# openclimatefix/graph_weather

Measured on AMD Instinct MI355X. Metric: forward forecasts/sec (1° grid, 102→78 feat), higher is better.
Workload: dtype f32; 1 GPU; c2: GraphWeatherForecaster 1deg grid (64800 nodes), 102->78 feat, batch=2 on rank 0, fp32, mesh res 2 (5882 nodes), random-init weights; global_batch=2, parallelism=batch-sharded x1, no collective in forward

## Files before the change

### graph_weather_amd/_lib.py

```python
from __future__ import annotations

import ctypes
import os
import subprocess
from ctypes import POINTER, Structure, c_char_p, c_float, c_int, c_int32, c_int64, c_size_t, c_void_p

_HERE = os.path.dirname(os.path.abspath(__file__))
CSRC = os.path.join(_HERE, "csrc")
LIB_PATH = os.path.join(CSRC, "libgw_amd.so")
HIPCC_FLAGS = ["--offload-arch=gfx950", "-O3", "-std=c++17", "-munsafe-fp-atomics", "-shared", "-fPIC"]

ABI_VERSION = 19
DTYPE_F32, DTYPE_BF16, DTYPE_BF16X3 = 0, 1, 2
LAYOUT_ROWS_F32, LAYOUT_EDGE_TILES_BF16, LAYOUT_ROWS_F16, LAYOUT_ROWS_BF16K = 0, 1, 2, 3
EDGE_DETERMINISTIC, EDGE_SEGMENT_TILES, EDGE_AGG_BF16K, EDGE_SEGMENT_SPLIT = 1, 2, 4, 8

EXPORTS = [
    "gw_version", "gw_last_error", "gw_debug_timestamps", "gw_packed_floats", "gw_pack_linear", "gw_packed_bytes_bf16",
    "gw_pack_linear_bf16", "gw_packed_bytes_bf16x3", "gw_pack_linear_bf16x3", "gw_padded_n", "gw_pad_vector", "gw_pack_many", "gw_mlp_chain_backward", "gw_mlp_chain_backward_bf16x3", "gw_mlp_ln_chain_backward",
    "gw_mlp_forward", "gw_mlp_post_forward", "gw_project_forward", "gw_edge_update_forward", "gw_edge_update_workspace_bytes", "gw_edge_tiles_bytes",
    "gw_edge_rows_to_tiles", "gw_node_update_forward", "gw_node_update_row_split_groups", "gw_node_update_head_forward",
    "gw_normalized_mse_forward", "gw_gemm_f32", "gw_relu_backward", "gw_layernorm_backward", "gw_gather_rows",
    "gw_segment_sum_rows", "gw_normalized_mse_backward", "gw_adamw_step", "gw_nudging_forward", "gw_nudging_backward",
    "gw_linear_forward", "gw_linear_gather_forward", "gw_layernorm_forward", "gw_add_rows", "gw_gather_rows_wide", "gw_segment_sum_rows_wide",
# ... 4 lines not shown
    "gw_thermal_rows",
    "gw_amse_mmax", "gw_amse_dft_rows", "gw_amse_legendre_floats", "gw_amse_coeff_floats", "gw_amse_workspace_bytes",
    "gw_amse_forward", "gw_amse_backward",
    "gw_modulate_workspace_bytes", "gw_sdl_forward", "gw_sdl_backward", "gw_film_forward", "gw_film_backward",
    "gw_attention_forward", "gw_attention_backward", "gw_knn_interpolate_forward", "gw_knn_interpolate_backward",
    "gw_gelu_forward", "gw_gelu_backward",
    "gw_attention_axial_forward", "gw_attention_axial_backward",
    "gw_patch_workspace_bytes", "gw_patch_embed_forward", "gw_patch_embed_backward", "gw_patch_expand_forward",
    "gw_patch_expand_backward",
    "gw_attention_masked_forward", "gw_attention_masked_backward",
    "gw_earth_loss_workspace_bytes", "gw_earth_loss_forward", "gw_earth_loss_backward",
    "gw_token_mean_forward", "gw_token_mean_backward", "gw_relu_forward", "gw_row_scale",
    "gw_conv3d_workspace_bytes", "gw_conv3d_forward", "gw_conv3d_backward",
    "gw_gemm_tn_ordered_workspace_bytes", "gw_gemm_tn_ordered", "gw_layernorm_backward_ordered_workspace_bytes",
    "gw_layernorm_backward_ordered",
    "gw_encoder_fused_forward",
    "gw_graph_attention_forward", "gw_graph_attention_backward", "gw_cond_layernorm_forward", "gw_cond_layernorm_backward",
    "gw_beta_gate_forward", "gw_beta_gate_workspace_bytes", "gw_beta_gate_backward", "gw_silu_forward", "gw_silu_backward",
    "gw_fourier_forward", "gw_fourier_backward",
    "gw_graph_attention_batched_forward", "gw_graph_attention_batched_backward", "gw_cond_layernorm_grouped_forward",
    "gw_cond_layernorm_grouped_workspace_bytes", "gw_cond_layernorm_grouped_backward", "gw_gencast_precond_input_forward",
    "gw_gencast_precond_input_backward", "gw_gencast_precond_output_forward", "gw_gencast_precond_output_backward",
    "gw_isht_lmax", "gw_isht_legendre_floats", "gw_isht_workspace_bytes", "gw_isht_forward",
    "gw_gencast_sampler_combine", "gw_gencast_weighted_mse_workspace_bytes", "gw_gencast_weighted_mse_forward",
    "gw_gencast_weighted_mse_backward",
    "gw_cond_layernorm_fanout_forward", "gw_cond_layernorm_fanout_workspace_bytes", "gw_cond_layernorm_fanout_backward",
    "gw_linear_gather_grouped_forward", "gw_segment_sum_rows_grouped",
]

GEMM_NN, GEMM_TN, GEMM_TN_BF16X3 = 0, 1, 2

# ... 145 lines not shown
    L.gw_edge_tiles_bytes.argtypes = [c_int32, c_int32]
    L.gw_edge_rows_to_tiles.restype = c_int
    L.gw_edge_rows_to_tiles.argtypes = [c_int32, c_int32, c_void_p, c_int32, c_int32, c_void_p, c_void_p]
    L.gw_edge_update_workspace_bytes.restype = c_size_t
    L.gw_edge_update_workspace_bytes.argtypes = [c_int32, c_int32, POINTER(GwOperand), POINTER(GwOperand), POINTER(GwOperand),
                                                 POINTER(GwMlpWeights), c_int32]
    L.gw_node_update_forward.restype = c_int
    L.gw_node_update_forward.argtypes = [c_int64, c_int32, POINTER(GwOperand), POINTER(GwOperand), POINTER(GwOperand),
                                         POINTER(GwMlpWeights), c_void_p, c_int32, POINTER(GwActivationSave), c_int32,
                                         POINTER(c_void_p), POINTER(c_void_p), c_int32, c_void_p, c_void_p]
    L.gw_node_update_row_split_groups.restype = c_int
    L.gw_node_update_row_split_groups.argtypes = [c_int64]
    L.gw_node_update_head_forward.restype = c_int
    L.gw_node_update_head_forward.argtypes = [c_int64, c_int32, POINTER(GwOperand), POINTER(GwOperand), POINTER(GwMlpWeights),
                                              POINTER(GwMlpWeights), POINTER(GwOperand), c_void_p, c_int32, c_void_p]
    L.gw_project_forward.restype = c_int
    L.gw_project_forward.argtypes = [c_int64, c_int32, POINTER(GwOperand), c_int32, POINTER(c_void_p), POINTER(c_void_p),
                                     c_int32, c_int32, c_int32, c_void_p, c_void_p, c_void_p]
    L.gw_normalized_mse_forward.restype = c_int
    L.gw_normalized_mse_forward.argtypes = [c_void_p, c_void_p, c_void_p, c_int32, c_void_p, c_int32, c_int32, c_int32, c_int32,
                                            c_void_p, c_void_p]
    L.gw_gemm_f32.restype = c_int
    L.gw_gemm_f32.argtypes = [c_int32, c_int64, c_int32, c_int64, c_void_p, c_int32, c_void_p, c_int32, c_void_p, c_int32, c_void_p,
                              c_void_p]
    L.gw_relu_backward.restype = c_int
    L.gw_relu_backward.argtypes = [c_int64, c_int32, c_void_p, c_int32, c_void_p, c_int32, c_void_p, c_int32, c_void_p, c_void_p]
    L.gw_layernorm_backward.restype = c_int
    L.gw_layernorm_backward.argtypes = [c_int64, c_int32, c_void_p, c_int32, c_void_p, c_int32, c_void_p, c_void_p, c_int32, c_void_p,
                                        c_void_p, c_void_p]
    L.gw_gather_rows.restype = c_int
# ... 264 lines not shown
```

### graph_weather_amd/layers.py

```python
from __future__ import annotations

from typing import List, Optional, Tuple

import torch
from torch import nn

from . import autograd as ag
from . import ops
from . import routes
from . import wide
from .autograd import OperandSpec
from .graphs import ForecastGraphs, GraphPlan, build_forecast_graphs
from .ops import BF16X3, Operand, PackedMLP
from .thermalizer import ThermalizerLayer

_NORMS = ["LayerNorm", "GraphNorm", "InstanceNorm", "BatchNorm", "MessageNorm"]


def _ver(t: torch.Tensor) -> int:
    return -1 if t.is_inference() else t._version


def _version_key(params) -> tuple:
    return tuple((p.data_ptr(), _ver(p), p.device) for p in params)
# ... 19 lines not shown
        hit = self._entries.get(name)
        if hit is None or hit[0] != key or hit[2] is not hold:
            hit = (key, make(), hold)
            self._entries[name] = hit
        return hit[1]

    def fresh(self, name: str, key, hold=None) -> bool:
        hit = self._entries.get(name)
        return hit is not None and hit[0] == key and hit[2] is hold

    def clear(self) -> None:
        self._entries.clear()

    def __contains__(self, name: str) -> bool:
        return name in self._entries


def _autograd_on(module: nn.Module, *inputs: Optional[torch.Tensor]) -> bool:
    on = torch.is_grad_enabled() and (any(p.requires_grad for p in module.parameters())
                                      or any(t is not None and t.requires_grad for t in inputs))
    if on:
        for m in module.modules():
            if isinstance(m, MLP) and m.compute_dtype == torch.bfloat16:
                raise NotImplementedError("graph_weather_amd: the backward pass is implemented for float32 and bf16x3 matrix "
                                          "products; call the bfloat16 mode under torch.no_grad() (inference)")
    return on


def _form(mlp: "MLP") -> routes.MlpForm:
    if mlp.compute_dtype == torch.bfloat16:
# ... 208 lines not shown
        self.node_mlp = MLP(in_dim_node + in_dim_edge, in_dim_node, hidden_dim, hidden_layers, norm_type).as_table()
        self.node_mlp.set_input_splits(((0, in_dim_node), (in_dim_node, in_dim_node + in_dim_edge)))


class GraphNetBlock(nn.Module):

    def __init__(self, edge_model: EdgeProcessor, node_model: NodeProcessor):
        super().__init__()
        self.edge_model = edge_model
        self.node_model = node_model
        self.deterministic = False

    def run(self, batch: int, plan: GraphPlan, x_src: Feed, x_dst: Feed, e_in: Feed, e_res: torch.Tensor, e_res_rows_pb: int,
            x_node: Feed, x_res: Optional[torch.Tensor], x_res_rows_pb: int, want_edges: bool, device,
            tag: Optional[str] = None, agg_zeroed: Optional[torch.Tensor] = None, post_w=None, post_zero: bool = False,
            post_half: bool = False, head=None, seg=None, agg_acc: Optional[torch.Tensor] = None):
        n_dst, n_edges = plan.n_dst, plan.num_edges
        if _autograd_on(self, x_src.tensor, x_dst.tensor, e_in.tensor, e_res, x_node.tensor, x_res):
            agg, e_out = ag.edge_update(self.edge_model.edge_mlp, plan, batch, (x_src.spec(), x_dst.spec(), e_in.spec()),
                                        want_edges, x_src.tensor, x_dst.tensor, e_in.tensor, e_res, e_res_rows_pb)
            x_new = ag.node_update(self.node_model.node_mlp, batch * n_dst, n_dst, x_node.spec(), x_node.tensor, x_res,
                                   x_res_rows_pb, agg)
            return x_new, e_out
        if seg is not None and agg_acc is not None:
            if want_edges not in (False, "tiles"):
                raise RuntimeError("graph_weather_amd: a processor block on segment-aligned tiles hands e' over as edge tiles")
            agg = agg_acc
            n_edges = seg.n_pad
        elif seg is not None:
            if want_edges or e_res is not None:
                raise RuntimeError("graph_weather_amd: segment-aligned tiles come without residual and without e'")
            if seg.split:
                agg = agg_zeroed if agg_zeroed is not None else torch.zeros((batch * n_dst, 256), dtype=torch.float32, device=device)
            else:
                agg = (torch.empty if seg.complete else torch.zeros)((batch * n_dst, 256), dtype=torch.bfloat16, device=device)
        else:
            agg = agg_zeroed if agg_zeroed is not None else torch.zeros((batch * n_dst, 256), dtype=torch.float32, device=device)
        if want_edges == "tiles":
            e_out = torch.empty(ops.edge_tiles_bytes(batch, n_edges), dtype=torch.uint8, device=device)
        else:
            e_out = torch.empty((batch * n_edges, 256), dtype=torch.float32, device=device) if want_edges else None
        res_op = ops.ZERO if e_res is None else Operand(e_res, e_res_rows_pb, 256, tiles=(e_res.dtype == torch.uint8))
        ops.edge_update_forward(self.edge_model.edge_mlp.packed(), batch, plan.src if seg is None else seg.src,
                                plan.dst if seg is None else seg.dst, x_src.operand(), x_dst.operand(),
                                e_in.operand(), res_op, n_dst, agg, e_out, tag=tag, deterministic=self.deterministic,
                                segment_tiles=seg is not None, segment_split=seg is not None and seg.split and agg_acc is None)
        res_x = ops.ZERO if x_res is None else Operand(x_res, x_res_rows_pb, 256)
        if head is not None:
            if x_res is not None:
                raise RuntimeError("graph_weather_amd: the fused node update + head has no node residual (decoder rows are zeros)")
            y = ops.node_update_head_forward(self.node_model.node_mlp.packed(), head[0], batch * n_dst, n_dst, x_node.operand(),
                                             Operand(agg, n_dst, 256), head[1])
            return y, e_out
        if post_w is not None:
            next_agg = torch.empty((batch * n_dst, 256), dtype=torch.float32, device=device) if post_zero else None
            if seg is not None and agg_acc is not None and not post_zero:
                next_agg = None
            x_new, posts = ops.node_update_forward(self.node_model.node_mlp.packed(), batch * n_dst, n_dst, x_node.operand(), res_x,
                                                   Operand(agg, n_dst, 256), post_w=post_w, zero_rows=next_agg, post_half=post_half)
            return x_new, e_out, posts, next_agg
        x_new = ops.node_update_forward(self.node_model.node_mlp.packed(), batch * n_dst, n_dst, x_node.operand(), res_x,
                                        Operand(agg, n_dst, 256))
        return x_new, e_out

    def params_key(self) -> tuple:
# ... 503 lines not shown
        self.efficient_batching = efficient_batching
        self.num_latlons = len(lat_lons)
        self.graphs = _graphs if _graphs is not None else build_forecast_graphs(lat_lons, resolution)
        self.num_h3 = self.graphs.num_mesh
        self.output_dim = output_dim
        self.edge_encoder = MLP(2, output_edge_dim, hidden_dim_processor_edge, 2, mlp_norm_type, use_checkpointing).as_table()
        self.graph_processor = GraphProcessor(mp_iterations=1, in_dim_node=input_dim, in_dim_edge=output_edge_dim,
                                              hidden_dim_node=hidden_dim_processor_node,
                                              hidden_dim_edge=hidden_dim_processor_edge,
                                              hidden_layers_node=hidden_layers_processor_node,
                                              hidden_layers_edge=hidden_layers_processor_edge, norm_type=mlp_norm_type,
                                              use_checkpointing=use_checkpointing)
        self.node_decoder = MLP(input_dim, output_dim, hidden_dim_decoder, hidden_layers_decoder, None, use_checkpointing)
        self._dev_plans = {}
        self._cache = KeyedCache()

    def _plan(self, device) -> GraphPlan:
        key = str(device)
        if key not in self._dev_plans:
            self._dev_plans[key] = self.graphs.dec_plan.to(device)
        return self._dev_plans[key]

    def edge_embedding(self, plan: GraphPlan) -> torch.Tensor:
        if _autograd_on(self):
            return self.edge_encoder.table(plan.edge_attr)
        return self._cache.get("dec_e", _version_key(list(self.edge_encoder.parameters())), lambda: self.edge_encoder.table(plan.edge_attr))

    def prefetch_tables(self, dev) -> Optional["torch.cuda.Stream"]:
        if wide.decoder_is_wide(self) or _autograd_on(self) or len(self.graph_processor.blocks) == 0:
            return None
# ... 44 lines not shown
            return False
        native = not mlp_e._layout()[4] and mlp_e._norm() is not None and len(mlp_e._linears()) == 3
        form = routes.MlpForm(torch.float32, 1 if native else -1, 0 if native else -1, native)
        return routes.decoder_stream(form, mlp_n.compute_dtype, self.graphs.dec_plan.num_edges, False, _autograd_on(self),
                                     bool(blk.deterministic), bool(ops.EDGE_STREAM))

    def _e_sum_product(self, plan: GraphPlan, e_rows: torch.Tensor, key, half: bool) -> torch.Tensor:
        pm_n = self.graph_processor.blocks[0].node_model.node_mlp.packed()
        n_e = plan.num_edges

        def make_e_sum():
            e_sum = ag.segment_sum_rows(e_rows, n_e, 1, 1, plan.n_dst, plan.dst_ptr(), None)
            return ops.project_forward([pm_n.w1[1]], Operand(e_sum, plan.n_dst, 256), plan.n_dst, plan.n_dst, out_half=half)[0]

        return self._cache.get("dec_e_sum", key, make_e_sum)

    def split_path(self) -> bool:
        return self._block_route() == routes.BLOCK_SPLIT

    def decode(self, processor_features: torch.Tensor, batch_size: int,
               residual: Optional[torch.Tensor] = None, ps: Optional[torch.Tensor] = None) -> torch.Tensor:
        B, G, M = batch_size, self.num_latlons, self.num_h3
        if processor_features.shape[0] != B * M:
            raise RuntimeError("processor_features must have batch*num_h3 rows")
        dev = processor_features.device
        if wide.decoder_is_wide(self):
            return wide.decode(self, processor_features, B, residual=residual)
        processor_features = _pad256(processor_features)
        plan = self._plan(dev)
        e = self.edge_embedding(plan)
# ... 31 lines not shown
        res = None
        if residual is not None:
            if residual.dim() != 2 or residual.shape[0] != B * G or residual.shape[1] < self.output_dim:
                raise RuntimeError("graph_weather_amd: the residual (start features) must have batch*num_latlons rows of at least "
                                   "output_dim = %d features, got %s" % (self.output_dim, tuple(residual.shape)))
            res = Operand(residual, G, self.output_dim)
        head = None
        if not train:
            nd = self.node_decoder
            if nd.compute_dtype == blk.node_model.node_mlp.compute_dtype and not wide.is_wide(nd) and not nd._layout()[4]:
                pm_h = nd.packed()
                pm_nn = blk.node_model.node_mlp.packed()
                if (pm_h.hidden == 128 and pm_h.n_mid == 1 and pm_h.n_out <= 80 and pm_h.gamma is None and pm_nn.n_mid == 1
                        and pm_nn.gamma is not None and pm_nn.ln_width == 0):
                    head = (pm_h, res)
        if not train and x_node is not FEED_ZERO:
            out, _ = blk.run(B, plan, Feed(ps, M, "proj"), FEED_ZERO, Feed(pe, 0, "proj"), None, 0, x_node, None, 0, False, dev,
                             tag="decoder_edge", head=head, seg=seg)
            if head is not None:
                return out.reshape(B, G, self.output_dim)
            xg = out
        elif head is not None and mlp_e.compute_dtype == torch.float32:
            out, _ = blk.run(B, plan, Feed(ps, M, "proj"), FEED_ZERO, Feed(pe, 0, "proj"), e, 0, FEED_ZERO, None, 0, False, dev,
                             tag="decoder_edge", head=head)
            return out.reshape(B, G, self.output_dim)
        else:
            xg, _ = blk.run(B, plan, Feed(ps, M, "proj"), FEED_ZERO, Feed(pe, 0, "proj"), e, 0, FEED_ZERO, None, 0, False, dev,
                            tag="decoder_edge")
        y = self.node_decoder.run(xg, B * G, G, residual=res)
        if y.shape[1] != self.output_dim:
            y = y[:, :self.output_dim]
        return y.reshape(B, G, self.output_dim)

    def forward(self, processor_features: torch.Tensor, batch_size: int) -> torch.Tensor:
        return self.decode(processor_features, batch_size)


def fused_forward(encoder: "Encoder", processor: "Processor", decoder: "AssimilatorDecoder", features: torch.Tensor,
                  residual: torch.Tensor, t=0) -> torch.Tensor:
# ... 77 lines not shown
```

### graph_weather_amd/ops.py

```python
from __future__ import annotations

from dataclasses import dataclass
from typing import List, Optional, Sequence, Tuple

import torch

from . import _lib
from ._lib import GwActivationSave, GwMlpWeights, GwOperand


class KernelTimer:

    def __init__(self, tags):
        self.tags = set(tags)
        self.events = {t: [] for t in self.tags}
        self.units = {t: [] for t in self.tags}

    def start(self, tag):
        if tag not in self.tags:
            return None
        ev = (torch.cuda.Event(enable_timing=True), torch.cuda.Event(enable_timing=True))
        ev[0].record()
        return ev

# ... 11 lines not shown
        evs = self.events[tag]
        return sum(a.elapsed_time(b) for a, b in evs) / max(1, len(evs))


TIMER: Optional[KernelTimer] = None

EDGE_STREAM = True
"""float32 inference: the decoder's edge update runs without the per-edge residual on the decoder-form kernel of
csrc/gw_edge_stream.hip (the segment sums of the batch-shared edge embedding enter the node update as a cached product).
``False`` forces the per-edge residual route on ``edge_kernel`` (csrc/gw_edge.hip).  Read on every ``decode``."""

ENCODER_FUSED = True
"""float32 inference: the encoder's node encoder and edge update run as ONE launch (csrc/gw_encoder_fused.hip) that keeps the
grid rows in registers and adds no per-edge residual (the segment sums of the batch-shared edge embedding enter the node update
as a cached product).  ``False`` keeps the two launches (``chain_kernel`` + ``elds_kernel``).  Read on every ``encode``."""


def _stream(t: torch.Tensor) -> int:
    return torch.cuda.current_stream(t.device).cuda_stream


class _NoGuard:
    def __enter__(self):
        return None

    def __exit__(self, *exc):
        return False


_NO_GUARD = _NoGuard()
# ... 358 lines not shown
def node_update_head_forward(pm: PackedMLP, head: PackedMLP, n_rows: int, rows_per_batch: int, x: Operand, agg: Operand,
                             residual: Optional[Operand], out: Optional[torch.Tensor] = None) -> torch.Tensor:
    if out is None:
        out = torch.empty((n_rows, head.n_out), dtype=torch.float32, device=agg.tensor.device)
    _require(out, "out")
    wc = pm.c((x.k > 0 and not x.projected, True, False))
    rc = residual.c() if residual is not None else None
    if rc is not None:
        rc.k = head.n_out
    with on_device_of(out):
        _lib.check(_lib.lib().gw_node_update_head_forward(n_rows, rows_per_batch, x.c(), agg.c(), wc, head.c(), rc, out.data_ptr(),
                                                          int(out.stride(0)), _stream(out)), "gw_node_update_head_forward")
    return out


def normalized_mse_forward(pred: torch.Tensor, target: torch.Tensor, lat_weights: torch.Tensor,
                           inv_var: Optional[torch.Tensor]) -> torch.Tensor:
    _require(pred, "pred")
    _require(target, "target")
    _require(lat_weights, "lat_weights")
    if pred.shape != target.shape or pred.dim() < 3:
        raise RuntimeError("graph_weather_amd: pred/target must both be [B, nodes..., C]")
    b = int(pred.shape[0])
    c = int(pred.shape[-1])
    nodes = pred.numel() // (b * c)
    full = 0
    if inv_var is not None:
        _require(inv_var, "inv_var")
        if inv_var.numel() == pred.numel():
            full = 1
# ... 268 lines not shown
```

### graph_weather_amd/routes.py

```python
from __future__ import annotations

from dataclasses import dataclass
from typing import Optional, Sequence, Tuple

import torch

BF16X3 = "bf16x3"



@dataclass(frozen=True)
class MlpForm:

    dtype: object
    n_mid: int
    ln_width: int
    has_norm: bool

    @staticmethod
    def of(mlp, packed=None) -> "MlpForm":
        pm = mlp.packed() if packed is None else packed
        return MlpForm(mlp.compute_dtype, int(pm.n_mid), int(pm.ln_width), pm.gamma is not None)


# ... 39 lines not shown
        return BLOCK_ROWS
    if edge.dtype == BF16X3 and node_dtype == BF16X3:
        return BLOCK_SPLIT
    if edge.dtype == torch.bfloat16 and node_dtype == torch.bfloat16 and not deterministic and resident_bf16(edge, n_edges):
        return BLOCK_TEAM
    return BLOCK_ROWS


def decoder_stream(edge: MlpForm, node_dtype, n_edges: int, wide: bool, autograd: bool, deterministic: bool, enabled: bool) -> bool:
    if not enabled or wide or autograd or deterministic or n_edges <= 0:
        return False
    return (edge.dtype == torch.float32 and node_dtype == torch.float32 and edge.n_mid == 1 and edge.ln_width == 0
            and edge.has_norm)


def encoder_fused(node_enc: MlpForm, node_enc_k: int, edge: MlpForm, node_dtype, n_edges: int, num_latlons: int, wide: bool,
                  autograd: bool, deterministic: bool, enabled: bool) -> bool:
    if not enabled or wide or autograd or deterministic or n_edges <= 0 or n_edges != num_latlons:
        return False
    if not (node_enc.dtype == torch.float32 and node_enc.n_mid == 1 and node_enc.ln_width == 0 and node_enc.has_norm
            and 16 < node_enc_k <= 112):
        return False
    return (edge.dtype == torch.float32 and node_dtype == torch.float32 and edge.n_mid == 1 and edge.ln_width == 0
            and edge.has_norm)




def stack_on_segment_tiles(blocks: Sequence[Tuple[MlpForm, object, bool]], n_edges: int, max_slots: Optional[int]) -> bool:
    if len(blocks) == 0 or n_edges <= 0 or max_slots is None or max_slots > 16:
# ... 32 lines not shown
```

### include/gw_amd.h

```cpp
#ifndef GW_AMD_H
#define GW_AMD_H

#include <stddef.h>
#include <stdint.h>

#ifdef __cplusplus
extern "C" {
#endif

#define GW_OK 0
#define GW_E_BADARG (-1)
#define GW_E_UNSUPPORTED (-2)
#define GW_E_LAUNCH (-3)

#define GW_ABI_VERSION 19

#define GW_DTYPE_F32 0
#define GW_DTYPE_BF16 1
#define GW_DTYPE_BF16X3 2

#define GW_LAYOUT_ROWS_F32 0
#define GW_LAYOUT_EDGE_TILES_BF16 1
#define GW_LAYOUT_ROWS_F16 2
#define GW_LAYOUT_ROWS_BF16K 3
// ... 113 lines not shown
                             const gw_mlp_weights* w_edge, float* agg , int32_t n_dst,
                             const struct gw_activation_save* save , int32_t flags , void* stream);

int gw_node_update_forward(int64_t n_rows, int32_t rows_per_batch, const gw_operand* x, const gw_operand* x_res,
                           const gw_operand* agg, const gw_mlp_weights* w, float* x_out, int32_t out_ld,
                           const struct gw_activation_save* save ,
                           int32_t n_post , const float* const* post_w, void* const* post_out,
                           int32_t post_layout ,
                           float* zero_rows , void* stream);

int gw_node_update_row_split_groups(int64_t n_rows);

int gw_node_update_head_forward(int64_t n_rows, int32_t rows_per_batch, const gw_operand* x, const gw_operand* agg,
                                const gw_mlp_weights* w, const gw_mlp_weights* head, const gw_operand* residual ,
                                float* out, int32_t out_ld, void* stream);

int gw_normalized_mse_forward(const float* pred, const float* target,
                              const float* inv_var ,
                              int32_t inv_var_full, const float* lat_weights, int32_t num_unique_lat, int32_t batch, int32_t nodes,
                              int32_t channels, float* loss_out, void* stream);


typedef struct gw_activation_save {
  float* hidden;
  int64_t hidden_stride;
  int32_t hidden_ld;
  float* pre_norm;
} gw_activation_save;

#define GW_GEMM_NN 0
// ... 308 lines not shown
```

Measured before the change: 316.4 forecasts/s.

## Add fused decoder node-update+head kernel that clears a persistent aggregate buffer

Adds a new HIP kernel that runs the decoder node MLP, LayerNorm and the output head in one launch, with constants staged in LDS and weights streamed through a double-buffered LDS ring. After reading its aggregate rows, the kernel zeroes them. This lets the decoder keep one zeroed aggregate buffer across forwards instead of allocating and zero-filling a 64800x2x256 fp32 buffer each call. The cost is a persistent per-stream buffer and a correctness dependency on every forward clearing it, including under graph capture.

After: 318.8 forecasts/s (median of 6 runs). No clear change (+0.8%).

```diff
diff --git a/graph_weather_amd/_lib.py b/graph_weather_amd/_lib.py
--- a/graph_weather_amd/_lib.py
+++ b/graph_weather_amd/_lib.py
@@ -42,7 +42,7 @@
     "gw_conv3d_workspace_bytes", "gw_conv3d_forward", "gw_conv3d_backward",
     "gw_gemm_tn_ordered_workspace_bytes", "gw_gemm_tn_ordered", "gw_layernorm_backward_ordered_workspace_bytes",
     "gw_layernorm_backward_ordered",
-    "gw_encoder_fused_forward",
+    "gw_encoder_fused_forward", "gw_node_head_stream_forward",
     "gw_graph_attention_forward", "gw_graph_attention_backward", "gw_cond_layernorm_forward", "gw_cond_layernorm_backward",
     "gw_beta_gate_forward", "gw_beta_gate_workspace_bytes", "gw_beta_gate_backward", "gw_silu_forward", "gw_silu_backward",
     "gw_fourier_forward", "gw_fourier_backward",
@@ -218,6 +218,9 @@
     L.gw_node_update_head_forward.restype = c_int
     L.gw_node_update_head_forward.argtypes = [c_int64, c_int32, POINTER(GwOperand), POINTER(GwOperand), POINTER(GwMlpWeights),
                                               POINTER(GwMlpWeights), POINTER(GwOperand), c_void_p, c_int32, c_void_p]
+    L.gw_node_head_stream_forward.restype = c_int
+    L.gw_node_head_stream_forward.argtypes = [c_int64, c_int32, POINTER(GwOperand), POINTER(GwOperand), POINTER(GwMlpWeights),
+                                              POINTER(GwMlpWeights), POINTER(GwOperand), c_void_p, c_int32, c_void_p, c_void_p]
     L.gw_project_forward.restype = c_int
     L.gw_project_forward.argtypes = [c_int64, c_int32, POINTER(GwOperand), c_int32, POINTER(c_void_p), POINTER(c_void_p),
                                      c_int32, c_int32, c_int32, c_void_p, c_void_p, c_void_p]
diff --git a/graph_weather_amd/csrc/gw_node_head.hip b/graph_weather_amd/csrc/gw_node_head.hip
--- /dev/null
+++ b/graph_weather_amd/csrc/gw_node_head.hip
@@ -0,0 +1,441 @@
+
+#include <hip/hip_runtime.h>
+#include <stdint.h>
+#include <string.h>
+
+#include "gw_device.hpp"
+#include "gw_edge_common.hpp"
+#include "gw_internal.hpp"
+
+using namespace gw;
+
+namespace {
+
+constexpr int kNodeSet = 0, kHeadSet = kConstSetFloats;
+constexpr int kNheadLdsBytes = (kConstOff + 2 * kConstSetFloats) * 4;
+static_assert(kNheadLdsBytes == 77056, "weight ring / staging area (66 560) + ids (256) + constants (10 240)");
+static_assert(2 * kNheadLdsBytes <= 160 * 1024, "two workgroups per CU must fit the 160 KiB of LDS");
+static_assert(kChunkFloats == kLdsBufFloats, "every chunk of the ring is a full LDS buffer");
+
+struct NheadArgs {
+  int n_cols;
+  int rows_pb;
+  int stagger;
+  int xcd_base;
+  int xcd_rem;
+  const float* agg;
+  int agg_rows_pb;
+  const float* p_ptr;
+  int p_rows_pb;
+  int p_ld;
+  const float* w_a;
+  const float* w_mid;
+  const float* w_out;
+  const float* n_const[5];
+  const float* hd_w1;
+  const float* hd_w2;
+  const float* hd_w3;
+  const float* hd_b[3];
+  const float* res_ptr;
+  int res_rows_pb;
+  int res_ld;
+  float* out;
+  int out_ld;
+  int out_cols;
+};
+
+constexpr int kHeadChunk0 = 3 * kChunksPerLayer;
+constexpr int kChunksPerTile = kHeadChunk0 + 4 + 2 + 2;
+
+__device__ __forceinline__ const float* chunk_src(const NheadArgs& a, int i) {
+  if (i < kHeadChunk0) {
+    const float* m = i < 8 ? a.w_a : (i < 16 ? a.w_mid : a.w_out);
+    return m + (size_t)(i & 7) * kChunkFloats;
+  }
+  i -= kHeadChunk0;
+  if (i < 4) return a.hd_w1 + (size_t)i * kChunkFloats;
+  if (i < 6) return a.hd_w2 + (size_t)(i - 4) * kChunkFloats;
+  return a.hd_w3 + (size_t)(i - 6) * kChunkFloats;
+}
+
+typedef float f32x2 __attribute__((ext_vector_type(2)));
+__device__ __forceinline__ f32x2 hld2(const float* p) {
+  f32x2 v;
+  asm volatile("global_load_dwordx2 %0, %1, off" : "=v"(v) : "v"(p) : "memory");
+  return v;
+}
+template <int N>
+__device__ __forceinline__ void wait_const(float (&c)[8]) {
+  asm volatile("s_waitcnt vmcnt(%[n])"
+               : "+v"(c[0]), "+v"(c[1]), "+v"(c[2]), "+v"(c[3]), "+v"(c[4]), "+v"(c[5]), "+v"(c[6]), "+v"(c[7])
+               : [n] "n"(N)
+               : "memory");
+}
+__device__ __forceinline__ void wait_pairs(f32x2 (&r)[10]) {
+  asm volatile("s_waitcnt vmcnt(0)"
+               : "+v"(r[0]), "+v"(r[1]), "+v"(r[2]), "+v"(r[3]), "+v"(r[4]), "+v"(r[5]), "+v"(r[6]), "+v"(r[7]), "+v"(r[8]), "+v"(r[9])
+               :
+               : "memory");
+}
+__device__ __forceinline__ void wait_singles(float (&r)[20]) {
+  asm volatile("s_waitcnt vmcnt(0)"
+               : "+v"(r[0]), "+v"(r[1]), "+v"(r[2]), "+v"(r[3]), "+v"(r[4]), "+v"(r[5]), "+v"(r[6]), "+v"(r[7]), "+v"(r[8]), "+v"(r[9]),
+                 "+v"(r[10]), "+v"(r[11]), "+v"(r[12]), "+v"(r[13]), "+v"(r[14]), "+v"(r[15]), "+v"(r[16]), "+v"(r[17]), "+v"(r[18]),
+                 "+v"(r[19])
+               :
+               : "memory");
+}
+
+#define GW_NCHUNK(ACC, NT, IN, OFF, NS, NP, DS, NNT, WAIT_STMT)                                                \
+  {                                                                                                            \
+    constexpr int nt4_ = ((NT) + 3) / 4, nnt4_ = ((NNT) + 3) / 4;                                              \
+    const float* bl_ = lds + (ci & 1) * kLdsBufFloats + lane * 4;                                              \
+    const float* nsrc_ = chunk_src(a, (NP) > 0 ? ci + 1 : ci);                                                 \
+    _Pragma("unroll") for (int s_ = 0; s_ < (NS); ++s_) {                                                      \
+      f32x4 a_nxt_[4];                                                                                         \
+      if ((NP) > 0 && s_ < (DS))                                                                               \
+        issue_pieces<((NP) > 0 ? (NP) / (DS) : 1)>(nsrc_, ((ci + 1) & 1) * kLdsBufFloats, s_ * ((NP) / (DS)), lane, wave); \
+      if (s_ + 1 < (NS)) {                                                                                     \
+        _Pragma("unroll") for (int b4 = 0; b4 < nt4_; ++b4)                                                    \
+            a_nxt_[b4] = *(const f32x4*)(bl_ + (s_ + 1) * (nt4_ * 256) + b4 * 256);                            \
+      } else if ((NP) > 0) {                                                                                   \
+        WAIT_STMT;                                                                                             \
+        lds_barrier();                                                                                         \
+        const float* bn_ = lds + ((ci + 1) & 1) * kLdsBufFloats + lane * 4;                                    \
+        _Pragma("unroll") for (int b4 = 0; b4 < nnt4_; ++b4) a_nxt_[b4] = *(const f32x4*)(bn_ + b4 * 256);      \
+      }                                                                                                        \
+      const float b_ = IN[(OFF) + s_];                                                                         \
+      __builtin_amdgcn_sched_barrier(0);                                                                       \
+      _Pragma("unroll") for (int t = 0; t < (NT); ++t)                                                         \
+          ACC[t] = __builtin_amdgcn_mfma_f32_16x16x4f32(a_cur[t >> 2][t & 3], b_, ACC[t], 0, 0, 0);             \
+      __builtin_amdgcn_sched_barrier(0);                                                                       \
+      if (s_ + 1 < (NS)) {                                                                                     \
+        _Pragma("unroll") for (int b4 = 0; b4 < nt4_; ++b4) a_cur[b4] = a_nxt_[b4];                             \
+      } else if ((NP) > 0) {                                                                                   \
+        _Pragma("unroll") for (int b4 = 0; b4 < nnt4_; ++b4) a_cur[b4] = a_nxt_[b4];                            \
+      }                                                                                                        \
+    }                                                                                                          \
+    ++ci;                                                                                                      \
+  }
+
+template <bool PROJ, bool CLEAR>
+__global__ __launch_bounds__(kThreads, 2) void nodehead_kernel(const NheadArgs a) {
+  float* const lds = lds_base();
+  const float* const cst = lds + kConstOff;
+  constexpr int NPROJ = 1;
+  GW_TILE_COORDS(a.n_cols, a.rows_pb, 0, 0)
+  stagger_start(a.stagger);
+
+  float cv[8];
+  {
+    const int f = threadIdx.x;
+#pragma unroll
+    for (int i = 0; i < 5; ++i) cv[i] = hld1(a.n_const[i] + f);
+    cv[5] = hld1(a.hd_b[0] + (f & 127));
+    cv[6] = hld1(a.hd_b[1] + (f & 127));
+    cv[7] = hld1(a.hd_b[2] + (f < 80 ? f : 0));
+  }
+  issue_chunk32k(chunk_src(a, 0), lds, lane, wave);
+  int ci = 0;
+  const float* xrow = a.agg + ((size_t)b * (size_t)a.agg_rows_pb + (size_t)k) * 256 + 4 * q;
+  f32x4 xv[16];
+  hld_row(xv, xrow);
+  wait_const<8 + 16>(cv);
+  consts_to_lds(lds, kNodeSet, cv);
+  {
+    float* cw = lds + kConstOff + kHeadSet + threadIdx.x;
+    cw[kB1] = cv[5];
+    cw[kBMid] = cv[6];
+    cw[kBOut] = cv[7];
+  }
+  const float* prow[NPROJ];
+  prow[0] = PROJ ? a.p_ptr + ((size_t)b * (size_t)a.p_rows_pb + (size_t)k) * (size_t)a.p_ld + 4 * q : xrow;
+
+  f32x4 ring[2][NPROJ][2];
+#define GW_CONSUME_SLICE(slot, slice)                                          \
+  {                                                                            \
+    f32x4 v0_ = acc[(2 * (slice)) & 15], v1_ = acc[(2 * (slice) + 1) & 15];    \
+    if (PROJ) {                                                                \
+      v0_ += ring[slot][0][0];                                                 \
+      v1_ += ring[slot][0][1];                                                 \
+    }                                                                          \
+    _Pragma("unroll") for (int r = 0; r < 4; ++r) {                            \
+      in8[r] = fmaxf(v0_[r], 0.f);                                             \
+      in8[4 + r] = fmaxf(v1_[r], 0.f);                                         \
+    }                                                                          \
+  }
+
+  f32x4 a_cur[4];
+  f32x4 acc[16];
+  f32x4 acc2[16];
+  float in8[8];
+  f32x4 o[16];
+  {
+    wait_regs<0>(xv);
+    lds_barrier();
+#pragma unroll
+    for (int t = 0; t < 16; ++t) acc[t] = *(const f32x4*)(cst + kNodeSet + kB1 + 16 * t + 4 * q);
+#pragma unroll
+    for (int b4 = 0; b4 < 4; ++b4) a_cur[b4] = *(const f32x4*)(lds + lane * 4 + b4 * 256);
+    float x[64];
+#pragma unroll
+    for (int i = 0; i < 16; ++i) {
+      x[4 * i + 0] = xv[i].x;
+      x[4 * i + 1] = xv[i].y;
+      x[4 * i + 2] = xv[i].z;
+      x[4 * i + 3] = xv[i].w;
+    }
+#pragma unroll
+    for (int cc = 0; cc < kChunksPerLayer; ++cc) {
+      if (PROJ && cc == kChunksPerLayer - 3) {
+        GW_REQUEST_SLICE(0, 0)
+        GW_REQUEST_SLICE(1, 1)
+      }
+      if (cc == kChunksPerLayer - 1) {
+#pragma unroll
+        for (int t = 0; t < 16; ++t) acc2[t] = *(const f32x4*)(cst + kNodeSet + kBMid + 16 * t + 4 * q);
+      }
+      GW_NCHUNK(acc, 16, x, 8 * cc, 8, 8, 4, 16, wait_vm<0>())
+    }
+    if (PROJ) {
+      wait_regs<0>(ring[0]);
+      wait_regs<0>(ring[1]);
+    }
+    GW_CONSUME_SLICE(0, 0)
+    if (PROJ) GW_REQUEST_SLICE(0, 2)
+  }
+
+#define GW_PRODUCE_CHUNK(cc)                                                                  \
+  {                                                                                           \
+    if (PROJ && (cc) <= 6) {                                                                  \
+      GW_NCHUNK(acc2, 16, in8, 0, 8, 8, 4, 16, wait_regs<0>(ring[((cc) + 1) & 1]))             \
+    } else {                                                                                  \
+      GW_NCHUNK(acc2, 16, in8, 0, 8, 8, 4, 16, wait_vm<0>())                                   \
+    }                                                                                         \
+    if ((cc) + 1 < kChunksPerLayer) GW_CONSUME_SLICE(((cc) + 1) & 1, (cc) + 1)                 \
+  }
+  GW_PRODUCE_CHUNK(0)
+  if (PROJ) GW_REQUEST_SLICE(1, 3)
+  GW_PRODUCE_CHUNK(1)
+  if (PROJ) GW_REQUEST_SLICE(0, 4)
+  GW_PRODUCE_CHUNK(2)
+  if (PROJ) GW_REQUEST_SLICE(1, 5)
+  GW_PRODUCE_CHUNK(3)
+  if (PROJ) GW_REQUEST_SLICE(0, 6)
+  GW_PRODUCE_CHUNK(4)
+  if (PROJ) GW_REQUEST_SLICE(1, 7)
+  GW_PRODUCE_CHUNK(5)
+  GW_PRODUCE_CHUNK(6)
+  GW_PRODUCE_CHUNK(7)
+
+  {
+    float hin[64];
+#pragma unroll
+    for (int t = 0; t < 16; ++t)
+#pragma unroll
+      for (int r = 0; r < 4; ++r) hin[4 * t + r] = fmaxf(acc2[t][r], 0.f);
+#pragma unroll
+    for (int t = 0; t < 16; ++t) o[t] = *(const f32x4*)(cst + kNodeSet + kBOut + 16 * t + 4 * q);
+#pragma unroll
+    for (int cc = 0; cc < kChunksPerLayer; ++cc) {
+      if (cc + 1 < kChunksPerLayer) {
+        GW_NCHUNK(o, 16, hin, 8 * cc, 8, 8, 4, 16, wait_vm<0>())
+      } else {
+        GW_NCHUNK(o, 16, hin, 8 * cc, 8, 8, 4, 8, wait_vm<0>())
+      }
+    }
+  }
+  GW_LAYERNORM256(o, GW_LDS4, cst + kNodeSet + kGamma, cst + kNodeSet + kBeta, )
+
+  f32x4 h1[8];
+  {
+    float xin[64];
+#pragma unroll
+    for (int t = 0; t < 16; ++t)
+#pragma unroll
+      for (int r = 0; r < 4; ++r) xin[4 * t + r] = o[t][r];
+#pragma unroll
+    for (int t = 0; t < 8; ++t) h1[t] = *(const f32x4*)(cst + kHeadSet + kB1 + 16 * t + 4 * q);
+#pragma unroll
+    for (int cc = 0; cc < 4; ++cc) GW_NCHUNK(h1, 8, xin, 16 * cc, 16, 8, 8, 8, wait_vm<0>())
+  }
+  f32x4 h2[8];
+  {
+    float hin1[32];
+#pragma unroll
+    for (int t = 0; t < 8; ++t) h2[t] = *(const f32x4*)(cst + kHeadSet + kBMid + 16 * t + 4 * q);
+#pragma unroll
+    for (int cc = 0; cc < 2; ++cc) {
+#pragma unroll
+      for (int t = 4 * cc; t < 4 * cc + 4; ++t)
+#pragma unroll
+        for (int r = 0; r < 4; ++r) hin1[4 * t + r] = fmaxf(h1[t][r], 0.f);
+      if (cc == 0) {
+        GW_NCHUNK(h2, 8, hin1, 16 * cc, 16, 8, 8, 8, wait_vm<0>())
+      } else {
+        GW_NCHUNK(h2, 8, hin1, 16 * cc, 16, 8, 8, 5, wait_vm<0>())
+      }
+    }
+  }
+  const float* rrow = a.res_ptr ? a.res_ptr + ((size_t)b * (size_t)a.res_rows_pb + (size_t)k) * (size_t)a.res_ld : nullptr;
+  float* orow = a.out + (size_t)c * (size_t)a.out_ld;
+  const bool pairs = (a.out_cols & 1) == 0 && ((size_t)orow & 7) == 0 && ((size_t)rrow & 7) == 0;
+  f32x2 rp[10];
+  float rs[20];
+  if (rrow) {
+    if (pairs) {
+#pragma unroll
+      for (int t = 0; t < 5; ++t)
+#pragma unroll
+        for (int r = 0; r < 4; r += 2) {
+          const int f = 16 * t + 4 * q + r;
+          rp[2 * t + (r >> 1)] = hld2(rrow + (f < a.out_cols ? f : 0));
+        }
+    } else {
+#pragma unroll
+      for (int t = 0; t < 5; ++t)
+#pragma unroll
+        for (int r = 0; r < 4; ++r) {
+          const int f = 16 * t + 4 * q + r;
+          rs[4 * t + r] = hld1(rrow + (f < a.out_cols ? f : 0));
+        }
+    }
+  }
+  f32x4 y[5];
+  {
+    float hin2[32];
+#pragma unroll
+    for (int t = 0; t < 8; ++t)
+#pragma unroll
+      for (int r = 0; r < 4; ++r) hin2[4 * t + r] = fmaxf(h2[t][r], 0.f);
+#pragma unroll
+    for (int t = 0; t < 5; ++t) y[t] = *(const f32x4*)(cst + kHeadSet + kBOut + 16 * t + 4 * q);
+    GW_NCHUNK(y, 5, hin2, 0, 16, 8, 8, 5, wait_vm<0>())
+    GW_NCHUNK(y, 5, hin2, 16, 16, 0, 1, 5, wait_vm<0>())
+  }
+
+  if (rrow) {
+    if (pairs) wait_pairs(rp); else wait_singles(rs);
+  }
+  if (valid) {
+#pragma unroll
+    for (int t = 0; t < 5; ++t) {
+      const int f0 = 16 * t + 4 * q;
+      if (pairs) {
+#pragma unroll
+        for (int r = 0; r < 4; r += 2)
+          if (f0 + r < a.out_cols) {
+            f32x2 v = f32x2{y[t][r], y[t][r + 1]};
+            if (rrow) {
+              const f32x2 rv = rp[2 * t + (r >> 1)];
+              v.x += rv.x;
+              v.y += rv.y;
+            }
+            *(GW_AS1 f32x2*)(orow + f0 + r) = v;
+          }
+      } else {
+#pragma unroll
+        for (int r = 0; r < 4; ++r)
+          if (f0 + r < a.out_cols) stg1(orow + f0 + r, y[t][r] + (rrow ? rs[4 * t + r] : 0.f));
+      }
+    }
+  }
+  if (CLEAR) {
+    const size_t rowp = (size_t)(a.agg + ((size_t)b * (size_t)a.agg_rows_pb + (size_t)k) * 256);
+    const unsigned lo = (unsigned)rowp, hi = (unsigned)(rowp >> 32);
+    const int n_here = a.n_cols - (tile_c0 + wave * kColsPerWave);
+#pragma unroll
+    for (int r = 0; r < kColsPerWave; ++r) {
+      if (r < n_here) {
+        float* zrow = (float*)(((size_t)(unsigned)__builtin_amdgcn_readlane((int)hi, r) << 32) | (size_t)(unsigned)__builtin_amdgcn_readlane((int)lo, r));
+        stg4(zrow + 4 * lane, f32x4{0.f, 0.f, 0.f, 0.f});
+      }
+    }
+  }
+#undef GW_CONSUME_SLICE
+#undef GW_PRODUCE_CHUNK
+}
+
+int unsupported(const char* msg) { return set_error(GW_E_UNSUPPORTED, msg); }
+
+}
+
+int gw_node_head_stream_forward(int64_t n_rows, int32_t rows_per_batch, const gw_operand* x, const gw_operand* agg,
+                                const gw_mlp_weights* w, const gw_mlp_weights* head, const gw_operand* residual, float* out,
+                                int32_t out_ld, float* clear_rows, void* stream) {
+  if (!x || !agg || !w || !head || !out || n_rows < 0 || rows_per_batch <= 0)
+    return set_error(GW_E_BADARG, "gw_node_head_stream_forward: bad arguments");
+  if (clear_rows != nullptr && clear_rows != agg->ptr)
+    return set_error(GW_E_BADARG, "gw_node_head_stream_forward: clear_rows must be NULL or the aggregate itself");
+  if (n_rows == 0) return GW_OK;
+  if (n_rows >= (int64_t)1 << 31) return unsupported("gw_node_head_stream_forward: more than 2^31-1 rows");
+  if (w->weight_dtype != GW_DTYPE_F32 || head->weight_dtype != GW_DTYPE_F32)
+    return unsupported("gw_node_head_stream_forward: float32 weights in both MLPs");
+  if (w->hidden != 256 || w->n_out != 256 || !w->b1 || !w->w_mid || !w->b_mid || !w->w_out || !w->b_out || w->n_mid != 1 ||
+      !w->ln_gamma || !w->ln_beta || (w->ln_width > 0 && w->ln_width != 256))
+    return unsupported("gw_node_head_stream_forward: node MLP must be 512 -> 256 -> 256 -> 256 with one middle layer and LayerNorm "
+                       "over 256 features");
+  if (agg->k != 256 || !agg->ptr || agg->projected || agg->index || agg->layout != GW_LAYOUT_ROWS_F32 || agg->ld != 256 || !w->w1[1])
+    return unsupported("gw_node_head_stream_forward: agg must be raw fp32 rows of 256 floats (ld 256, no index)");
+  if (x->k != 0 && (x->k != 256 || !x->ptr || !x->projected || x->index || x->layout != GW_LAYOUT_ROWS_F32 || x->ld % 4 != 0))
+    return unsupported("gw_node_head_stream_forward: x must be projected 256-wide fp32 rows or absent (k = 0)");
+  if (head->hidden != 128 || head->n_mid != 1 || head->n_out > 80 || head->n_out <= 0 || head->ln_gamma || !head->w1[0] || !head->b1 ||
+      !head->w_mid || !head->b_mid || !head->w_out || !head->b_out)
+    return unsupported("gw_node_head_stream_forward: the head must be 256 -> 128 -> 128 -> <= 80 features without norm");
+  if (head->k_in != 256 || (head->out_rows != 80 && !(head->out_rows == 0 && head->n_out == 80)))
+    return unsupported("gw_node_head_stream_forward: the head must be packed for 256 inputs (k_in) and 80 output rows (out_rows)");
+  const bool res = residual && residual->k != 0;
+  if (res && (!residual->ptr || residual->layout != GW_LAYOUT_ROWS_F32))
+    return set_error(GW_E_BADARG, "gw_node_head_stream_forward: bad residual");
+  if (res && residual->index) return unsupported("gw_node_head_stream_forward: the residual rows are not indexed");
+
+  static const int impl = GW_TUNE("GW_NODE_HEAD_STREAM", 1);
+  if (impl == 0) {
+    if (int rc = gw_node_update_head_forward(n_rows, rows_per_batch, x, agg, w, head, residual, out, out_ld, stream)) return rc;
+    if (clear_rows != nullptr && hipMemsetAsync(clear_rows, 0, (size_t)n_rows * 256 * sizeof(float), (hipStream_t)stream) != hipSuccess)
+      return set_error(GW_E_LAUNCH, "gw_node_head_stream_forward: hipMemsetAsync failed");
+    return GW_OK;
+  }
+
+  NheadArgs a;
+  memset(&a, 0, sizeof(a));
+  a.n_cols = (int)n_rows;
+  a.rows_pb = rows_per_batch;
+  a.agg = agg->ptr;
+  a.agg_rows_pb = agg->rows_per_batch;
+  const bool proj = x->k != 0;
+  if (proj) {
+    a.p_ptr = x->ptr;
+    a.p_rows_pb = x->rows_per_batch;
+    a.p_ld = x->ld;
+  }
+  a.w_a = w->w1[1];
+  a.w_mid = w->w_mid;
+  a.w_out = w->w_out;
+  a.n_const[0] = w->b1;
+  a.n_const[1] = w->b_mid;
+  a.n_const[2] = w->b_out;
+  a.n_const[3] = w->ln_gamma;
+  a.n_const[4] = w->ln_beta;
+  a.hd_w1 = head->w1[0];
+  a.hd_w2 = head->w_mid;
+  a.hd_w3 = head->w_out;
+  a.hd_b[0] = head->b1;
+  a.hd_b[1] = head->b_mid;
+  a.hd_b[2] = head->b_out;
+  if (res) {
+    a.res_ptr = residual->ptr;
+    a.res_rows_pb = residual->rows_per_batch;
+    a.res_ld = residual->ld;
+  }
+  a.out = out;
+  a.out_ld = out_ld;
+  a.out_cols = head->n_out;
+  fill_tile_schedule(a, (a.n_cols + kColsPerWG - 1) / kColsPerWG, 4);
+  const char* what = "nodehead_kernel launch";
+  if (clear_rows != nullptr)
+    return proj ? launch_tile_kernel(nodehead_kernel<true, true>, a, kNheadLdsBytes, what, stream)
+                : launch_tile_kernel(nodehead_kernel<false, true>, a, kNheadLdsBytes, what, stream);
+  return proj ? launch_tile_kernel(nodehead_kernel<true, false>, a, kNheadLdsBytes, what, stream)
+              : launch_tile_kernel(nodehead_kernel<false, false>, a, kNheadLdsBytes, what, stream);
+}
diff --git a/graph_weather_amd/layers.py b/graph_weather_amd/layers.py
--- a/graph_weather_amd/layers.py
+++ b/graph_weather_amd/layers.py
@@ -57,6 +57,22 @@
 
     def __contains__(self, name: str) -> bool:
         return name in self._entries
+
+
+class KeptAggregate:
+
+    def __init__(self, tensor: torch.Tensor):
+        self.tensor = tensor
+        self.dirty = False
+
+    def acquire(self) -> torch.Tensor:
+        if self.dirty:
+            self.tensor.zero_()
+        self.dirty = True
+        return self.tensor
+
+    def release(self) -> None:
+        self.dirty = False
 
 
 def _autograd_on(module: nn.Module, *inputs: Optional[torch.Tensor]) -> bool:
@@ -295,7 +311,8 @@
     def run(self, batch: int, plan: GraphPlan, x_src: Feed, x_dst: Feed, e_in: Feed, e_res: torch.Tensor, e_res_rows_pb: int,
             x_node: Feed, x_res: Optional[torch.Tensor], x_res_rows_pb: int, want_edges: bool, device,
             tag: Optional[str] = None, agg_zeroed: Optional[torch.Tensor] = None, post_w=None, post_zero: bool = False,
-            post_half: bool = False, head=None, seg=None, agg_acc: Optional[torch.Tensor] = None):
+            post_half: bool = False, head=None, seg=None, agg_acc: Optional[torch.Tensor] = None, head_stream: bool = False,
+            agg_kept: Optional[KeptAggregate] = None):
         n_dst, n_edges = plan.n_dst, plan.num_edges
         if _autograd_on(self, x_src.tensor, x_dst.tensor, e_in.tensor, e_res, x_node.tensor, x_res):
             agg, e_out = ag.edge_update(self.edge_model.edge_mlp, plan, batch, (x_src.spec(), x_dst.spec(), e_in.spec()),
@@ -315,6 +332,10 @@
                 agg = agg_zeroed if agg_zeroed is not None else torch.zeros((batch * n_dst, 256), dtype=torch.float32, device=device)
             else:
                 agg = (torch.empty if seg.complete else torch.zeros)((batch * n_dst, 256), dtype=torch.bfloat16, device=device)
+        elif agg_kept is not None:
+            if not (head_stream and head is not None):
+                raise RuntimeError("graph_weather_amd: a kept aggregate needs the launch that clears it (node update + head)")
+            agg = agg_kept.acquire()
         else:
             agg = agg_zeroed if agg_zeroed is not None else torch.zeros((batch * n_dst, 256), dtype=torch.float32, device=device)
         if want_edges == "tiles":
@@ -330,6 +351,12 @@
         if head is not None:
             if x_res is not None:
                 raise RuntimeError("graph_weather_amd: the fused node update + head has no node residual (decoder rows are zeros)")
+            if head_stream:
+                y = ops.node_head_stream_forward(self.node_model.node_mlp.packed(), head[0], batch * n_dst, n_dst, x_node.operand(),
+                                                 Operand(agg, n_dst, 256), head[1], clear=agg_kept is not None)
+                if agg_kept is not None:
+                    agg_kept.release()
+                return y, e_out
             y = ops.node_update_head_forward(self.node_model.node_mlp.packed(), head[0], batch * n_dst, n_dst, x_node.operand(),
                                              Operand(agg, n_dst, 256), head[1])
             return y, e_out
@@ -863,6 +890,7 @@
         self.node_decoder = MLP(input_dim, output_dim, hidden_dim_decoder, hidden_layers_decoder, None, use_checkpointing)
         self._dev_plans = {}
         self._cache = KeyedCache()
+        self._agg_cache = KeyedCache()
 
     def _plan(self, device) -> GraphPlan:
         key = str(device)
@@ -937,6 +965,18 @@
             return ops.project_forward([pm_n.w1[1]], Operand(e_sum, plan.n_dst, 256), plan.n_dst, plan.n_dst, out_half=half)[0]
 
         return self._cache.get("dec_e_sum", key, make_e_sum)
+
+    def kept_aggregate(self, batch: int, device) -> Optional[KeptAggregate]:
+        dev = torch.device(device)
+        on_gpu = dev.type == "cuda"
+        last = "dec_agg_last/%d/%s" % (int(batch), dev)
+        if on_gpu and torch.cuda.is_current_stream_capturing():
+            return self._agg_cache._entries[last][1] if last in self._agg_cache else None
+        stream = torch.cuda.current_stream(dev).cuda_stream if on_gpu else 0
+        kept = self._agg_cache.get("dec_agg/%d/%s/%d" % (int(batch), dev, stream), None, lambda: KeptAggregate(
+            torch.zeros((int(batch) * self.num_latlons, 256), dtype=torch.float32, device=dev)))
+        self._agg_cache.get(last, id(kept), lambda: kept)
+        return kept
 
     def split_path(self) -> bool:
         return self._block_route() == routes.BLOCK_SPLIT
@@ -998,15 +1038,20 @@
                 if (pm_h.hidden == 128 and pm_h.n_mid == 1 and pm_h.n_out <= 80 and pm_h.gamma is None and pm_nn.n_mid == 1
                         and pm_nn.gamma is not None and pm_nn.ln_width == 0):
                     head = (pm_h, res)
+        mlp_n = blk.node_model.node_mlp
+        head_stream = head is not None and routes.decoder_node_head_stream(
+            routes.MlpForm.of(mlp_n, pm_nn), self.node_decoder.compute_dtype, True, False, False, bool(blk.deterministic),
+            bool(ops.NODE_HEAD_STREAM))
+        kept = self.kept_aggregate(B, dev) if head_stream else None
         if not train and x_node is not FEED_ZERO:
             out, _ = blk.run(B, plan, Feed(ps, M, "proj"), FEED_ZERO, Feed(pe, 0, "proj"), None, 0, x_node, None, 0, False, dev,
-                             tag="decoder_edge", head=head, seg=seg)
+                             tag="decoder_edge", head=head, seg=seg, head_stream=head_stream, agg_kept=kept)
             if head is not None:
                 return out.reshape(B, G, self.output_dim)
             xg = out
         elif head is not None and mlp_e.compute_dtype == torch.float32:
             out, _ = blk.run(B, plan, Feed(ps, M, "proj"), FEED_ZERO, Feed(pe, 0, "proj"), e, 0, FEED_ZERO, None, 0, False, dev,
-                             tag="decoder_edge", head=head)
+                             tag="decoder_edge", head=head, head_stream=head_stream, agg_kept=kept)
             return out.reshape(B, G, self.output_dim)
         else:
             xg, _ = blk.run(B, plan, Feed(ps, M, "proj"), FEED_ZERO, Feed(pe, 0, "proj"), e, 0, FEED_ZERO, None, 0, False, dev,
diff --git a/graph_weather_amd/ops.py b/graph_weather_amd/ops.py
--- a/graph_weather_amd/ops.py
+++ b/graph_weather_amd/ops.py
@@ -49,6 +49,11 @@
 """float32 inference: the encoder's node encoder and edge update run as ONE launch (csrc/gw_encoder_fused.hip) that keeps the
 grid rows in registers and adds no per-edge residual (the segment sums of the batch-shared edge embedding enter the node update
 as a cached product).  ``False`` keeps the two launches (``chain_kernel`` + ``elds_kernel``).  Read on every ``encode``."""
+
+NODE_HEAD_STREAM = True
+"""float32 inference: the decoder's node update + output head runs on ``nodehead_kernel`` (csrc/gw_node_head.hip: constants in
+LDS) and clears the aggregate it has read, so the decoder keeps ONE zeroed aggregate buffer from forward to forward instead of
+filling a fresh one.  ``False`` keeps ``chain_kernel`` and the fill per forward.  Read on every ``decode``."""
 
 
 def _stream(t: torch.Tensor) -> int:
@@ -437,6 +442,22 @@
     return out
 
 
+def node_head_stream_forward(pm: PackedMLP, head: PackedMLP, n_rows: int, rows_per_batch: int, x: Operand, agg: Operand,
+                             residual: Optional[Operand], out: Optional[torch.Tensor] = None, clear: bool = False) -> torch.Tensor:
+    if out is None:
+        out = torch.empty((n_rows, head.n_out), dtype=torch.float32, device=agg.tensor.device)
+    _require(out, "out")
+    wc = pm.c((x.k > 0 and not x.projected, True, False))
+    rc = residual.c() if residual is not None else None
+    if rc is not None:
+        rc.k = head.n_out
+    with on_device_of(out):
+        _lib.check(_lib.lib().gw_node_head_stream_forward(n_rows, rows_per_batch, x.c(), agg.c(), wc, head.c(), rc, out.data_ptr(),
+                                                          int(out.stride(0)), agg.tensor.data_ptr() if clear else None,
+                                                          _stream(out)), "gw_node_head_stream_forward")
+    return out
+
+
 def normalized_mse_forward(pred: torch.Tensor, target: torch.Tensor, lat_weights: torch.Tensor,
                            inv_var: Optional[torch.Tensor]) -> torch.Tensor:
     _require(pred, "pred")
diff --git a/graph_weather_amd/routes.py b/graph_weather_amd/routes.py
--- a/graph_weather_amd/routes.py
+++ b/graph_weather_amd/routes.py
@@ -77,6 +77,14 @@
             and edge.has_norm)
 
 
+def decoder_node_head_stream(node: MlpForm, head_dtype, head_fused: bool, wide: bool, autograd: bool, deterministic: bool,
+                             enabled: bool) -> bool:
+    if not enabled or wide or autograd or deterministic or not head_fused:
+        return False
+    return (node.dtype == torch.float32 and head_dtype == torch.float32 and node.n_mid == 1 and node.ln_width == 0
+            and node.has_norm)
+
+
 def encoder_fused(node_enc: MlpForm, node_enc_k: int, edge: MlpForm, node_dtype, n_edges: int, num_latlons: int, wide: bool,
                   autograd: bool, deterministic: bool, enabled: bool) -> bool:
     if not enabled or wide or autograd or deterministic or n_edges <= 0 or n_edges != num_latlons:
diff --git a/include/gw_amd.h b/include/gw_amd.h
--- a/include/gw_amd.h
+++ b/include/gw_amd.h
@@ -151,6 +151,10 @@
 int gw_node_update_head_forward(int64_t n_rows, int32_t rows_per_batch, const gw_operand* x, const gw_operand* agg,
                                 const gw_mlp_weights* w, const gw_mlp_weights* head, const gw_operand* residual ,
                                 float* out, int32_t out_ld, void* stream);
+
+int gw_node_head_stream_forward(int64_t n_rows, int32_t rows_per_batch, const gw_operand* x, const gw_operand* agg,
+                                const gw_mlp_weights* w, const gw_mlp_weights* head, const gw_operand* residual ,
+                                float* out, int32_t out_ld, float* clear_rows , void* stream);
 
 int gw_normalized_mse_forward(const float* pred, const float* target,
                               const float* inv_var ,
```
